# PSeitz/lz4_flex

Measured on AMD Instinct MI355X. Metric: MiB/s compress+decompress round trip, 1 GiB of 64 KiB JSON blocks per GPU (LZ4 block format), higher is better.
Workload: dtype u8

## Files before the change

lz4_flex_amd/csrc/lz4_compress_wave.hip:

```cpp
#include <hip/hip_runtime.h>
#include <stdint.h>

#include "lz4_device.h"

namespace lz4flex_dev {
namespace wave {

typedef __attribute__((address_space(3))) uint8_t lds_u8;
typedef __attribute__((address_space(3))) uint16_t lds_u16;
typedef __attribute__((address_space(3))) uint32_t lds_u32;
typedef uint32_t u32x4 __attribute__((ext_vector_type(4)));
typedef __attribute__((address_space(1))) uint8_t g_u8;
typedef __attribute__((address_space(1))) u32x4 g_u32x4;
typedef uint32_t u32x2 __attribute__((ext_vector_type(2)));
typedef __attribute__((address_space(1))) u32x2 g_u32x2;
typedef __attribute__((address_space(1))) uint32_t g_u32;
typedef __attribute__((address_space(1))) int32_t g_i32;

constexpr uint32_t WINDOW = 65536u;
#ifndef LZ4W_WORKERS
#define LZ4W_WORKERS 11
#endif
constexpr uint32_t WORKERS = LZ4W_WORKERS;
constexpr uint32_t GROUPS = WINDOW / 512u;
__host__ __device__ constexpr uint32_t seg_lo(uint32_t w) {
    if (WORKERS == 11u) {
        constexpr uint32_t lo[12] = {0u, 12u, 25u, 38u, 51u, 63u, 74u, 86u, 98u, 108u, 118u, 128u};
        return 512u * lo[w < 11u ? w : 11u];
    }
    if (WORKERS == 8u) {
        constexpr uint32_t lo[9] = {0u, 16u, 33u, 50u, 67u, 82u, 98u, 113u, 128u};
        return 512u * lo[w < 8u ? w : 8u];
    }
    return 512u * ((GROUPS * w) / WORKERS);
}
__host__ __device__ constexpr uint32_t seg_longest() {
    uint32_t m = 0u;
    for (uint32_t w = 0u; w < WORKERS; ++w) m = seg_lo(w + 1u) - seg_lo(w) > m ? seg_lo(w + 1u) - seg_lo(w) : m;
    return m;
}
constexpr uint32_t SEG = seg_longest();
constexpr uint32_t HIST = WINDOW / 2u;
__device__ __forceinline__ uint32_t seg_start(uint32_t j, uint32_t skip, uint32_t send) {
    if (send == 0u) return seg_lo(j) > skip ? seg_lo(j) : skip;
    if (j == 0u) return skip;
    if (j >= WORKERS) return send;
    const uint32_t span = send > skip ? send - skip : 0u;
    const uint32_t v = (skip + span * (seg_lo(j) / 512u) / 128u) & ~511u;
    return v > skip ? v : skip;
}

constexpr uint32_t CAP = 1024u;
constexpr uint32_t SKIPD = 64u;
constexpr uint32_t CARRY_SLOTS = 16u;
constexpr uint32_t CARRY_DWORDS = CARRY_SLOTS * 16u;
constexpr uint32_t CARRY_SPINS = 1u << 18;
constexpr uint32_t LONGK = 84u;
constexpr uint32_t NEARP = 20u;
constexpr uint32_t LONGN = 8u;
constexpr uint32_t HBITS = 12u;
constexpr uint32_t THREADS = 64u * (WORKERS + 1u);
#ifndef LZ4W_RING_SLOTS
#define LZ4W_RING_SLOTS 1
#endif
constexpr uint32_t RING_SLOTS = LZ4W_RING_SLOTS;
constexpr uint32_t TMP_OFF = 16u;
constexpr uint32_t CMP_OFF = TMP_OFF + 256u;
constexpr uint32_t WORKER_LDS = CMP_OFF + 256u;
constexpr uint32_t CHUNK = 1024u;
constexpr uint32_t CHUNK_SLOT = CHUNK + 16u;
constexpr uint32_t IDX_DEPTH = 4u;
constexpr uint32_t L_WIN = 0u;
constexpr uint32_t L_TAB = WINDOW + 64u;
constexpr uint32_t L_STG = L_TAB + (2u << HBITS);
constexpr uint32_t L_RING = L_STG + WORKERS * WORKER_LDS;
constexpr uint32_t L_META = L_RING + RING_SLOTS * CHUNK_SLOT;
constexpr uint32_t META_WORDS = 5u * WORKERS + 4u + 4u + 3u + 2u;
constexpr uint32_t LDS_BYTES = L_META + ((META_WORDS * 4u + 63u) & ~63u);
static_assert(LDS_BYTES <= 81920u, "two workgroups per CU");
static_assert(WORKERS >= 1u && WORKERS <= 15u && seg_lo(WORKERS) == WINDOW, "segments tile the window");
constexpr uint32_t SLOT_BYTES = 2u * WINDOW;
constexpr uint32_t BODY_STRIDE = (SEG + SEG / 128u + 255u) / 256u * 256u + 256u;
constexpr uint32_t WS_BYTES = 2u * SLOT_BYTES + WORKERS * BODY_STRIDE;
static_assert(WS_BYTES % 256u == 0u, "workspace slots stay 256 B aligned");
constexpr uint32_t STAGE_BYTES = WINDOW + 256u;
constexpr uint32_t STAGE_READ = WINDOW + 64u;

struct SegMeta {
    uint32_t has;
    uint32_t first_lit;
    uint32_t first_ml;
    uint32_t trail;
    uint32_t body_len;
};
struct BlkCarry { uint32_t out_pos, pend; };

__device__ __forceinline__ uint32_t dpp_wave_shr1(uint32_t v, uint32_t lane0) {
    return (uint32_t)__builtin_amdgcn_update_dpp((int)lane0, (int)v, 0x138, 0xf, 0xf, false);
}
__device__ __forceinline__ uint32_t dpp_wave_shl1(uint32_t v, uint32_t lane63) {
    return (uint32_t)__builtin_amdgcn_update_dpp((int)lane63, (int)v, 0x130, 0xf, 0xf, false);
}
#define LZ4W_DPP(v, ctrl, rmask) ((uint32_t)__builtin_amdgcn_update_dpp(0, (int)(v), (ctrl), (rmask), 0xf, false))
__device__ __forceinline__ uint32_t wave_incl_max(uint32_t v) {
    uint32_t t;
    t = LZ4W_DPP(v, 0x111, 0xf); v = v > t ? v : t;
    t = LZ4W_DPP(v, 0x112, 0xf); v = v > t ? v : t;
    t = LZ4W_DPP(v, 0x114, 0xf); v = v > t ? v : t;
    t = LZ4W_DPP(v, 0x118, 0xf); v = v > t ? v : t;
    t = LZ4W_DPP(v, 0x142, 0xa); v = v > t ? v : t;
    t = LZ4W_DPP(v, 0x143, 0xc); v = v > t ? v : t;
    return v;
}
__device__ __forceinline__ uint32_t wave_incl_add(uint32_t v) {
    v += LZ4W_DPP(v, 0x111, 0xf);
    v += LZ4W_DPP(v, 0x112, 0xf);
    v += LZ4W_DPP(v, 0x114, 0xf);
    v += LZ4W_DPP(v, 0x118, 0xf);
    v += LZ4W_DPP(v, 0x142, 0xa);
    v += LZ4W_DPP(v, 0x143, 0xc);
    return v;
}
__device__ __forceinline__ uint32_t rdlane(uint32_t v, uint32_t l) { return (uint32_t)__builtin_amdgcn_readlane((int)v, (int)l); }
__device__ __forceinline__ uint32_t uni(uint32_t v) { return (uint32_t)__builtin_amdgcn_readfirstlane((int)v); }
__device__ __forceinline__ uint64_t ld64l(const lds_u8* p) { uint64_t v; __builtin_memcpy(&v, (const void*)p, 8); return v; }
__device__ __forceinline__ uint32_t umin3(uint32_t a, uint32_t b, uint32_t c) { const uint32_t t = a < b ? a : b; return t < c ? t : c; }
__device__ __forceinline__ uint32_t ctz64(uint64_t x) { return (uint32_t)__builtin_ctzll(x); }
__device__ __forceinline__ uint32_t len_ext_bytes(uint32_t v) { return v >= 15u ? (v - 15u) / 255u + 1u : 0u; }

#ifndef LZ4W_NO_HWFFBL
__device__ __forceinline__ uint32_t ffbl(uint32_t x) { uint32_t r; asm("v_ffbl_b32 %0, %1" : "=v"(r) : "v"(x)); return r; }
#else
__device__ __forceinline__ uint32_t ffbl(uint32_t x) { return (uint32_t)(__ffs((int)x) - 1); }
#endif
template <typename G, typename T>
__device__ __forceinline__ G* uni_gptr(T* p) {
    const uint64_t v = (uint64_t)p;
    return (G*)(((uint64_t)uni((uint32_t)(v >> 32)) << 32) | uni((uint32_t)v));
}

struct ChunkRegs { u32x4 main; uint32_t extra; };

__device__ __forceinline__ void chunk_issue(ChunkRegs& r, const g_u8* __restrict__ gwin, uint32_t c, uint32_t lane) {
    const g_u8* pm = gwin + c * CHUNK + 16u * lane;
    const g_u8* pe = gwin + c * CHUNK + CHUNK;
#ifdef LZ4W_PLAIN_LOADS
    r.main = *reinterpret_cast<const g_u32x4*>(pm);
    r.extra = *reinterpret_cast<const g_u32*>(pe);
#else
    asm volatile("global_load_dwordx4 %0, %1, off ; lz4w-load" : "=v"(r.main) : "v"(pm) : "memory");
    asm volatile("global_load_dword %0, %1, off ; lz4w-load" : "=v"(r.extra) : "v"(pe) : "memory");
#endif
}
template <int N>
__device__ __forceinline__ void chunk_wait(ChunkRegs& r) {
#ifndef LZ4W_PLAIN_LOADS
    asm volatile("s_waitcnt vmcnt(%2) ; lz4w-wait %0 %1" : "+v"(r.main), "+v"(r.extra) : "n"(N) : "memory");
#endif
}
template <bool FULL>
__device__ __forceinline__ void index_chunk(const lds_u8* lp, lds_u16* tab, g_u8* __restrict__ cand_lane, uint32_t c, uint32_t act_n,
                                            uint32_t lane) {
#pragma unroll
    for (uint32_t g8 = 0; g8 < 2u; ++g8) {
        uint32_t h[8], e[8];
        uint64_t xr[8];
// ... 737 lines not shown
    u32x2 dn = *reinterpret_cast<const g_u32x2*>(cand_t + ((s0 >> 8) * 512u + lane * 8u));
#ifndef LZ4W_NO_PRIO
    const uint32_t prio_q = (s1 - s0 + 3u) / 4u;
    uint32_t prio_drop = s0 + prio_q, prio_lv = 3u;
    __builtin_amdgcn_s_setprio(3);
#endif
    for (uint32_t B0 = s0 & ~255u; B0 < s1; B0 += 256u) {
        const uint32_t dq0 = dn.x & 0xFFFFu, dq1 = dn.x >> 16, dq2 = dn.y & 0xFFFFu, dq3 = dn.y >> 16;
        dn = *reinterpret_cast<const g_u32x2*>(cand_t + (((B0 >> 8) + 1u) * 512u + lane * 8u));
#ifndef LZ4W_NO_PRIO
        if (B0 >= prio_drop) {
            prio_drop += prio_q;
            prio_lv = prio_lv != 0u ? prio_lv - 1u : 0u;
            if (prio_lv == 2u) __builtin_amdgcn_s_setprio(2);
            else if (prio_lv == 1u) __builtin_amdgcn_s_setprio(1);
            else __builtin_amdgcn_s_setprio(0);
        }
#endif
        if (superstep(UConst<4u>{}, B0, dq0, dq1, dq2, dq3)) continue;
#pragma unroll 1
        for (uint32_t hf = 0u; hf < 2u; ++hf) {
            const uint32_t bh = B0 + 128u * hf;
            if (bh >= s1) break;
            const uint32_t ta = hf ? dq2 : dq0, tb = hf ? dq3 : dq1;
            superstep(UConst<2u>{}, bh, ta, tb, 0u, 0u);
        }
    }
    st = encode_seqs(psq, psp, npend, body_, lane, st);
#ifndef LZ4W_NO_PRIO
    __builtin_amdgcn_s_setprio(3);
#endif
#ifdef LZ4W_PROF_STEPS
    if (prof_ && lane == 0u) {
        for (int i = 0; i < 5; ++i) atomicAdd(prof_ + 8 + i, (unsigned long long)pt[i]);
        atomicAdd(prof_ + 13, (unsigned long long)pn);
        atomicAdd(prof_ + 14, (unsigned long long)pt[5]);
        atomicAdd(prof_ + 15, (unsigned long long)pt[6]);
    }
#endif
    if (lane == 0u) {
        lds_u32* mp = (lds_u32*)(lds + L_META) + 5u * w;
        mp[0] = st.has; mp[1] = st.first_lit; mp[2] = st.first_ml; mp[3] = s1 - st.last_end; mp[4] = st.body_len;
    }
}

template <typename F>
__device__ __forceinline__ void put_bytes(g_u8* dst, uint32_t n, uint32_t lane, F f) {
    for (uint32_t i = lane; i < n; i += 64u) dst[i] = (uint8_t)f(i);
}
__device__ __forceinline__ void copy_bytes(g_u8* dst, const g_u8* src, uint32_t n, uint32_t lane) {
    uint32_t i = 0u;
    for (; i + 4096u <= n; i += 4096u) {
        u32x4 v[4];
#pragma unroll
        for (uint32_t j = 0; j < 4u; ++j) __builtin_memcpy(&v[j], (const void*)(src + i + 1024u * j + 16u * lane), 16);
#pragma unroll
        for (uint32_t j = 0; j < 4u; ++j) __builtin_memcpy((void*)(dst + i + 1024u * j + 16u * lane), &v[j], 16);
    }
    {
        u32x4 v[4];
#pragma unroll
        for (uint32_t j = 0; j < 4u; ++j) {
            const uint32_t o = i + 1024u * j + 16u * lane;
            v[j] = u32x4{0u, 0u, 0u, 0u};
            if (o + 16u <= n) __builtin_memcpy(&v[j], (const void*)(src + o), 16);
        }
#pragma unroll
        for (uint32_t j = 0; j < 4u; ++j) {
            const uint32_t o = i + 1024u * j + 16u * lane;
            if (o + 16u <= n) __builtin_memcpy((void*)(dst + o), &v[j], 16);
        }
    }
    const uint32_t done = i + ((n - i) & ~15u);
    if (done + lane < n) dst[done + lane] = src[done + lane];
}
__device__ __forceinline__ void put_len_header(g_u8* dst, uint32_t lit, uint32_t ml_nibble, uint32_t lane) {
    const uint32_t ne = len_ext_bytes(lit);
    put_bytes(dst, 1u + ne, lane, [&](uint32_t j) -> uint32_t {
        if (j == 0u) return ((lit < 15u ? lit : 15u) << 4) | ml_nibble;
        return (j < ne) ? 255u : (lit - 15u) % 255u;
    });
}

__device__ __attribute__((noinline)) void place_segment(lds_u8* lds, const uint8_t* __restrict__ gin_, uint32_t blk_len_, uint32_t win_idx_, bool last_win_,
                              uint32_t wl_, uint32_t wbase_, uint32_t wskip_, uint32_t send_, const uint8_t* body_, uint8_t* gout_, uint32_t carry_slot_, uint32_t w_, uint32_t lane,
                              uint32_t* out_len_, int32_t* status_, uint32_t* gcarry_, uint32_t iter_, uint32_t spins_max_, uint32_t runwin_) {
    const g_u8* __restrict__ gin = uni_gptr<const g_u8>(gin_);
    const uint32_t runwin = uni(runwin_);
    const g_u8* body = uni_gptr<const g_u8>(body_);
    g_u8* gout = uni_gptr<g_u8>(gout_);
    g_u32* out_len = uni_gptr<g_u32>(out_len_);
    g_i32* status = uni_gptr<g_i32>(status_);
    const uint32_t blk_len = uni(blk_len_), win_idx = uni(win_idx_), wl = uni(wl_), carry_slot = uni(carry_slot_), w = uni(w_);
    const uint32_t wbase = uni(wbase_), wskip = uni(wskip_);
    const uint32_t spins_max = uni(spins_max_);
    const bool last_win = uni((uint32_t)last_win_) != 0u;
    const uint32_t send = uni(send_);
    const lds_u32* mp = (const lds_u32*)(lds + L_META);
    lds_u32* cp = (lds_u32*)(lds + L_META) + 5u * WORKERS;
    g_u32* gcarry = uni_gptr<g_u32>(gcarry_);
    uint32_t out_pos = 0u, pend = 0u, poisoned = 0u;
    if (win_idx != 0u) {
        if (gcarry != nullptr) {
            const uint32_t iter = uni(iter_);
            typedef volatile __attribute__((address_space(3))) uint32_t lds_vu32;
            lds_vu32* box = (lds_vu32*)(lds + L_META) + 5u * WORKERS + 8u;
#ifndef LZ4W_NO_PRIO
            __builtin_amdgcn_s_setprio(0);
#endif
            if (w == WORKERS - 1u) {
                g_u32* sl = gcarry + 16u * (win_idx & (CARRY_SLOTS - 1u));
                uint32_t spins = 0u;
                while (__hip_atomic_load(sl + 2, __ATOMIC_ACQUIRE, __HIP_MEMORY_SCOPE_AGENT) != win_idx && ++spins < spins_max) __builtin_amdgcn_s_sleep(16);
                out_pos = __hip_atomic_load(sl, __ATOMIC_RELAXED, __HIP_MEMORY_SCOPE_AGENT);
                pend = __hip_atomic_load(sl + 1, __ATOMIC_RELAXED, __HIP_MEMORY_SCOPE_AGENT);
                if (spins >= spins_max) pend = 0x80000000u;
                if (lane == 0u) { box[0] = out_pos; box[1] = pend; }
                __builtin_amdgcn_fence(__ATOMIC_RELEASE, "workgroup");
                if (lane == 0u) box[2] = iter;
            } else {
                uint32_t spins = 0u;
                while (box[2] != iter && ++spins < (CARRY_SPINS << 4)) __builtin_amdgcn_s_sleep(2);
                __builtin_amdgcn_fence(__ATOMIC_ACQUIRE, "workgroup");
                out_pos = box[0];
                pend = spins >= (CARRY_SPINS << 4) ? 0x80000000u : box[1];
            }
#ifndef LZ4W_NO_PRIO
            __builtin_amdgcn_s_setprio(3);
#endif
            poisoned = pend >> 31;
            pend &= 0x7FFFFFFFu;
            if (poisoned) { out_pos = 0u; pend = 0u; }
            out_pos = uni(out_pos); pend = uni(pend); poisoned = uni(poisoned);
        } else {
            out_pos = cp[2u * (carry_slot ^ 1u)]; pend = cp[2u * (carry_slot ^ 1u) + 1u];
        }
    }
    auto seg_at = [&](uint32_t j) -> uint32_t {
        const uint32_t v = runwin ? (j == 0u ? wskip : wl) : seg_start(j, wskip, send);
        return v < wl ? v : wl;
    };
    auto seg_len = [&](uint32_t j) -> uint32_t { return seg_at(j + 1u) - seg_at(j); };
    for (uint32_t j = 0; j < w; ++j) {
        const uint32_t sl = seg_len(j);
        if (mp[5u * j] != 0u) {
            const uint32_t L = pend + mp[5u * j + 1u];
            out_pos += 1u + len_ext_bytes(L) + L + mp[5u * j + 4u];
            pend = mp[5u * j + 3u];
        } else {
            pend += sl;
        }
    }
    const uint32_t sl = seg_len(w);
    const uint32_t abs0 = wbase + seg_at(w);
    if (gcarry != nullptr && w == WORKERS - 1u && !last_win && lane == 0u) {
        uint32_t eo = out_pos, ep = pend;
        if (mp[5u * w] != 0u) {
            const uint32_t L = pend + mp[5u * w + 1u];
            eo += 1u + len_ext_bytes(L) + L + mp[5u * w + 4u];
            ep = mp[5u * w + 3u];
        } else {
            ep += sl;
        }
        g_u32* so = gcarry + 16u * ((win_idx + 1u) & (CARRY_SLOTS - 1u));
        __hip_atomic_store(so, eo, __ATOMIC_RELAXED, __HIP_MEMORY_SCOPE_AGENT);
        __hip_atomic_store(so + 1, ep | (poisoned << 31), __ATOMIC_RELAXED, __HIP_MEMORY_SCOPE_AGENT);
        __hip_atomic_store(so + 2, win_idx + 1u, __ATOMIC_RELEASE, __HIP_MEMORY_SCOPE_AGENT);
    }
    if (mp[5u * w] != 0u) {
        const uint32_t fl = mp[5u * w + 1u], L = pend + fl, ml = mp[5u * w + 2u] - 4u, bl = mp[5u * w + 4u];
        put_len_header(gout + out_pos, L, ml < 15u ? ml : 15u, lane);
        out_pos += 1u + len_ext_bytes(L);
        copy_bytes(gout + out_pos, gin + (abs0 + fl - L), L, lane);
        out_pos += L;
        copy_bytes(gout + out_pos, body, bl, lane);
        out_pos += bl;
        pend = mp[5u * w + 3u];
    } else {
        pend += sl;
    }
    if (w == WORKERS - 1u) {
        if (last_win) {
            put_len_header(gout + out_pos, pend, 0u, lane);
            out_pos += 1u + len_ext_bytes(pend);
            copy_bytes(gout + out_pos, gin + (blk_len - pend), pend, lane);
            out_pos += pend;
            if (lane == 0u) { *out_len = poisoned ? 0u : out_pos; *status = poisoned ? 66  : 0; }
        } else if (lane == 0u) {
            cp[2u * carry_slot] = out_pos;
            cp[2u * carry_slot + 1u] = pend;
        }
    }
}

__device__ __attribute__((noinline)) void load_window(const uint8_t* __restrict__ g_, uint32_t wl_, uint32_t rd_n_, lds_u8* lds, uint32_t tid) {
    constexpr uint32_t NT = 64u * WORKERS;
    const g_u8* __restrict__ g = uni_gptr<const g_u8>(g_);
    const uint32_t wl = uni(wl_), rd_n = uni(rd_n_);
    const uint32_t mis = (uint32_t)((16u - ((uintptr_t)g & 15u)) & 15u);
    const uint32_t head = mis < wl ? mis : wl;
    if (tid < head) lds[L_WIN + tid] = g[tid];
    const uint32_t nvec = (wl - head) / 16u;
    const g_u8* gp = g + head + 16u * tid;
    lds_u8* lp = lds + L_WIN + head + 16u * tid;
#pragma unroll 1
    for (uint32_t i0 = 0; i0 < nvec; i0 += 4u * NT) {
        u32x4 v[4];
#pragma unroll
        for (uint32_t j = 0; j < 4u; ++j) {
            v[j] = u32x4{0u, 0u, 0u, 0u};
            if (i0 + tid + NT * j < nvec) v[j] = *reinterpret_cast<const g_u32x4*>(gp + 16u * NT * j);
        }
#pragma unroll
        for (uint32_t j = 0; j < 4u; ++j)
            if (i0 + tid + NT * j < nvec) __builtin_memcpy((void*)(lp + 16u * NT * j), &v[j], 16);
        gp += 64u * NT;
        lp += 64u * NT;
    }
    const uint32_t done = head + 16u * nvec;
    if (tid < wl - done) lds[L_WIN + done + tid] = g[done + tid];
    if (tid < 64u) lds[L_WIN + wl + tid] = wl + tid < rd_n ? g[wl + tid] : (uint8_t)0;
}

struct WaveArgs : CompressArgs {
    const uint8_t* shared_dict;
    uint32_t shared_len;
    uint32_t shared_hs;
    uint32_t shared_keep;
    uint8_t* digest;
};
template <class A> constexpr bool IS_SHARED = __is_same(A, WaveArgs);
struct SetArgs : CompressArgs {
    DictSetArgs set;
};
template <class A> constexpr bool IS_SET = __is_same(A, SetArgs);
template <class A> constexpr bool HAS_DIGEST = IS_SHARED<A> || IS_SET<A>;
struct Item {
    uint32_t blk, win, nwin, len, skip, hist, slide;
    uint32_t sub;
    uint32_t dct;
    uint32_t did;
    uint64_t in_off;
};
__device__ __forceinline__ uint32_t win_stride(const Item& t) { return t.slide != 0u ? t.slide : WINDOW; }
__device__ __forceinline__ uint32_t win_base(const Item& t) {
    if (t.sub != 0u) return 0u;
    return (t.win + 1u == t.nwin && t.len > WINDOW) ? t.len - WINDOW : t.win * win_stride(t);
}
__device__ __forceinline__ uint32_t win_from(const Item& t) {
    if (t.sub != 0u) return t.win * t.sub;
    return t.win == 0u ? t.hist : (t.win - 1u) * win_stride(t) + WINDOW;
}
__device__ __forceinline__ uint32_t win_skip(const Item& t) { return win_from(t) - win_base(t); }
__device__ __forceinline__ uint32_t win_len(const Item& t) {
    if (t.sub != 0u) return t.win + 1u == t.nwin ? t.len : (t.win + 1u) * t.sub;
    const uint32_t base = win_base(t);
    return t.len > base ? (t.len - base < WINDOW ? t.len - base : WINDOW) : 0u;
}
__device__ __forceinline__ uint32_t win_send(const Item& t) { return t.sub != 0u ? win_len(t) : (t.slide != 0u ? WINDOW : 0u); }
template <class A>
__device__ __forceinline__ void item_load(const A& a, Item& it) {
    it.win = 0u; it.nwin = 0u; it.len = 0u; it.skip = 0u; it.hist = 0u; it.slide = 0u; it.sub = 0u; it.dct = 0u; it.did = 0u; it.in_off = 0ull;
    if (it.blk >= a.n) return;
    const uint32_t len = a.in_len[it.blk];
    const uint32_t cap = a.out_cap[it.blk];
    uint32_t h = (a.flags != nullptr && (a.flags[it.blk] >> 8) >= HIST && len != 0u && len <= 0xFFFFFFFFu - HIST) ? HIST : 0u;
    uint32_t dl = a.dict_len != nullptr ? a.dict_len[it.blk] : 0u;
    if constexpr (IS_SHARED<A>) dl = a.shared_len;
    if constexpr (IS_SET<A>) {
        const uint32_t id = a.set.dict_id[it.blk];
        if (id != DICT_ID_NONE) {
            if (id >= a.set.k) { it.skip = 2u; it.nwin = 1u; return; }
            dl = a.set.table[id].len;
            it.did = id;
// ... 2 lines not shown
    if (dl != 0u) {
        h = dl < HIST ? dl : HIST;
        if ((a.flags != nullptr && a.flags[it.blk] != 0u) || len > 0xFFFFFFFFu - h) { it.skip = 2u; it.nwin = 1u; return; }
        it.dct = 1u;
    }
    it.hist = h;
    it.len = len + h;
    it.in_off = a.in_off[it.blk] - h;
    it.slide = h != 0u ? HIST : ((a.slide != 0u && len > WINDOW) ? a.slide : 0u);
    it.nwin = it.slide != 0u ? (it.len <= WINDOW ? 1u : 1u + (it.len - WINDOW + it.slide - 1u) / it.slide)
                      : (len == 0u ? 1u : (uint32_t)(((uint64_t)len + WINDOW - 1u) / WINDOW));
    if (a.sub >= 2u && a.sub <= 4u && h == 0u && len <= WINDOW) {
        const uint32_t q = ((WINDOW + a.sub - 1u) / a.sub + 511u) & ~511u;
        if (len > q) { it.sub = q; it.nwin = (len + q - 1u) / q; }
    }
    const uint64_t need = 20ull + (uint64_t)len * 110ull / 100ull;
    if ((uint64_t)cap < need) { it.skip = 1u; it.nwin = 1u; }
}
template <class A>
__device__ __forceinline__ const uint8_t* win_src(const A& a, const Item& t, const uint8_t* stg) {
    return t.dct ? stg : a.in_base + t.in_off + (size_t)win_base(t);
}
__device__ __forceinline__ uint32_t win_rd(const Item& t) {
    const uint32_t r = t.len - win_base(t);
    return t.dct && r > STAGE_READ ? STAGE_READ : r;
}
template <class A>
__device__ __forceinline__ void item_seek(const A& a, Item& it, int32_t redo) {
    if (redo != 0)
        while (it.blk < a.n && a.status[it.blk] != redo) it.blk += gridDim.x;
    item_load(a, it);
}
template <class A>
__device__ __forceinline__ void item_next_block(const A& a, Item& it, int32_t redo) {
    if (it.win + 1u < it.nwin) { it.win += 1u; return; }
    it.blk += gridDim.x;
    item_seek(a, it, redo);
}
template <class A>
__device__ __forceinline__ void item_draw(const A& a, uint32_t* wctr, uint32_t b0, uint32_t& ob, uint32_t& ow) {
    const uint32_t n = a.n;
    uint32_t b = b0;
    const uint32_t tries = n < 8u ? n : 8u;
    for (uint32_t t = 0; t < tries; ++t) {
        Item q;
        q.blk = b;
        item_load(a, q);
        const uint32_t w = atomicAdd(wctr + b, 1u);
        if (w < q.nwin) { ob = b; ow = w; return; }
        b = b + 1u == n ? 0u : b + 1u;
    }
    ob = n; ow = 0u;
}

struct RunGeom { uint32_t ok, ms, me; };
__device__ __forceinline__ RunGeom run_geom(const Item& t) {
    RunGeom g;
    const uint32_t base = win_base(t), wl = win_len(t), skip = win_skip(t);
    g.ms = skip > 1u ? skip : 1u;
    uint32_t me = t.len >= 5u + base ? t.len - 5u - base : 0u;
    me = me < wl ? me : wl;
    g.me = me < 65535u ? me : 65535u;
    const uint32_t act_abs = t.len >= 12u ? t.len - 11u : 0u;
#ifdef LZ4W_NO_RUN_WINDOWS
    g.ok = 0u;
#else
    g.ok = (wl >= RUN_MIN && !t.skip && base + g.ms < act_abs && g.me >= g.ms + 4u) ? 1u : 0u;
#endif
    return g;
}

__device__ __forceinline__ const uint8_t* item_digest(const WaveArgs& a, const Item&) { return a.digest; }
__device__ __forceinline__ uint32_t item_hs(const WaveArgs& a, const Item&) { return a.shared_hs; }
__device__ __forceinline__ uint32_t* item_counter(const WaveArgs& a) { return (uint32_t*)(a.digest + DG_HDR) + 2; }
__device__ __forceinline__ const DictSetRec* set_rec(const SetArgs& a, const Item& t) { return uni_gptr<const DictSetRec>(a.set.table) + uni(t.did); }
__device__ __forceinline__ const uint8_t* item_digest(const SetArgs& a, const Item& t) { return uni_gptr<const uint8_t>(set_rec(a, t)->digest); }
__device__ __forceinline__ uint32_t item_hs(const SetArgs& a, const Item& t) { return a.set.use != 0u ? uni(set_rec(a, t)->hs) : 0u; }
__device__ __forceinline__ uint32_t* item_counter(const SetArgs& a) { return a.set.counter; }
__device__ __forceinline__ uint32_t keep_tag(const WaveArgs& a, const Item&) { return a.shared_keep != 0u ? 1u : 0u; }
__device__ __forceinline__ bool keep_hit(const WaveArgs&, const Item&, uint32_t kept) { return kept != 0u; }
__device__ __forceinline__ uint32_t keep_tag(const SetArgs& a, const Item& t) { return a.set.use != 0u ? t.did + 1u : 0u; }
__device__ __forceinline__ bool keep_hit(const SetArgs&, const Item& t, uint32_t kept) { return kept == t.did + 1u; }

template <class A>
__device__ __forceinline__ void wave_body(const A& a, uint8_t* __restrict__ ws, uint32_t* __restrict__ carry,
                                          unsigned long long* __restrict__ prof, const int32_t redo, const uint32_t carry_spins) {
    extern __shared__ __attribute__((aligned(16))) uint8_t dyn_lds[];
    lds_u8* lds = (lds_u8*)dyn_lds;
    if ((uint32_t)(uintptr_t)lds != 0u) {
        for (uint32_t b = blockIdx.x * THREADS + threadIdx.x; b < a.n; b += gridDim.x * THREADS) { a.out_len[b] = 0u; a.status[b] = 66; }
        return;
    }
    const uint32_t lane = threadIdx.x & 63u;
    const uint32_t w = uni(threadIdx.x >> 6);
#ifdef LZ4W_EXP_IDX_PRIO
    if (w == WORKERS) __builtin_amdgcn_s_setprio(LZ4W_EXP_IDX_PRIO);
#endif
    uint8_t* my_ws = ws + (size_t)blockIdx.x * WS_BYTES;
    uint8_t* slots = my_ws;
    uint8_t* bodies = my_ws + 2u * SLOT_BYTES;
    uint8_t* stg = a.stage + (size_t)blockIdx.x * STAGE_BYTES;

    const bool wmode = carry != nullptr;
    lds_u32* giq = (lds_u32*)(lds + L_META) + 5u * WORKERS + 4u;
    uint32_t* wctr = wmode ? carry + CARRY_DWORDS * (size_t)a.n : nullptr;
    Item it, ix;
    if (threadIdx.x == 0u) giq[6] = 0u;
    if (wmode) {
        if (threadIdx.x == 0u) {
            uint32_t b = a.n, wn = 0u;
            item_draw(a, wctr, blockIdx.x % a.n, b, wn);
            giq[0] = b; giq[1] = wn;
        }
        __syncthreads();
        it.blk = giq[0];
        item_load(a, it);
        it.win = giq[1];
        ix.blk = a.n;
        item_load(a, ix);
    } else {
        it.blk = blockIdx.x;
        item_seek(a, it, redo);
        ix = it;
        item_next_block(a, ix, redo);
    }
    if (it.blk >= a.n) return;
    uint32_t k = 0u;

    lds_u32* run_flag = (lds_u32*)(lds + L_META) + 5u * WORKERS + 11u;
    [[maybe_unused]] uint32_t tail_kept = 0u;
    auto do_stage = [&](const Item& t) {
        const uint32_t base = win_base(t);
        const uint32_t nrd = win_rd(t);
        if constexpr (HAS_DIGEST<A>) {
            const uint32_t from = (t.win == 0u && keep_hit(a, t, tail_kept)) ? (t.hist & ~15u) : 0u;
            stage_window(item_digest(a, t) + DG_TAIL, a.in_base + t.in_off, base + from, nrd - from, t.hist, stg + from, lane);
            tail_kept = t.win == 0u ? keep_tag(a, t) : 0u;
            return;
        } else {
        const uint8_t* tail = a.dict_base + a.dict_off[t.blk] + (a.dict_len[t.blk] - t.hist);
        stage_window(tail, a.in_base + t.in_off, base, nrd, t.hist, stg, lane);
        }
    };
    auto do_index = [&](const Item& t, uint32_t slot, bool stage) {
        if (t.skip) { if (lane == 0u) run_flag[slot] = 0u; return; }
        if (t.dct && stage) do_stage(t);
        const uint32_t base = win_base(t), wl = win_len(t);
        const uint32_t act_abs = t.len >= 12u ? t.len - 11u : 0u;
        const uint32_t act_n = act_abs > base ? (act_abs - base < wl ? act_abs - base : wl) : 0u;
        const RunGeom rg = run_geom(t);
        if constexpr (HAS_DIGEST<A>) {
            const uint32_t hs = (IS_SHARED<A> || t.dct != 0u) ? item_hs(a, t) : 0u;
            if (t.win == 0u && hs != 0u && act_n >= hs) {
                const uint32_t run = index_window<true>(win_src(a, t, stg), wl, act_n, win_rd(t), slots + (size_t)slot * SLOT_BYTES, lds, lane, rg.ok,
                                                        DigestRef<true>{item_digest(a, t), hs});
                if (redo == 0 && lane == 0u)
                    __hip_atomic_fetch_add(item_counter(a), 1u, __ATOMIC_RELAXED, __HIP_MEMORY_SCOPE_AGENT);
                if (lane == 0u) run_flag[slot] = run;
                return;
            }
        }
        const uint32_t run = index_window<false>(win_src(a, t, stg), wl, act_n, win_rd(t), slots + (size_t)slot * SLOT_BYTES, lds, lane, rg.ok, DigestRef<false>{});
        if (lane == 0u) run_flag[slot] = run;
    };
    auto do_load = [&](const Item& t) {
        if (t.skip) return;
        load_window(win_src(a, t, stg), win_len(t), win_rd(t), lds, threadIdx.x);
    };

    uint64_t t_prev = prof ? __builtin_readcyclecounter() : 0ull;
    uint64_t t_acc[7] = {0ull, 0ull, 0ull, 0ull, 0ull, 0ull, 0ull};
    auto tick = [&](uint32_t slot) {
        if (prof) {
            const uint64_t t = __builtin_readcyclecounter();
#pragma unroll
            for (uint32_t i = 0; i < 7u; ++i) t_acc[i] += i == slot ? t - t_prev : 0ull;
            t_prev = t;
        }
    };
    if (it.dct && !it.skip) {
        if (w == WORKERS) do_stage(it);
        __syncthreads();
    }
    if (w == WORKERS) { do_index(it, 0u, false); tick(0u); }
    else { do_load(it); tick(5u); }
    __syncthreads();
    tick(w == WORKERS ? 1u : 6u);
    if (wmode) {
        if (threadIdx.x == 0u) {
            uint32_t b2 = a.n, w2 = 0u;
            item_draw(a, wctr, it.blk, b2, w2);
            giq[2] = b2; giq[3] = w2;
        }
        __syncthreads();
        ix.blk = giq[2];
        item_load(a, ix);
        ix.win = giq[3];
        __syncthreads();
    }
    for (;;) {
        const uint32_t wl = win_len(it);
        const bool last_win = it.win + 1u == it.nwin;
        if (w == WORKERS) {
            if (ix.blk < a.n) do_index(ix, (k + 1u) & 1u, true);
        } else if (!it.skip) {
            const uint32_t base = win_base(it), skip = win_skip(it);
            uint32_t s0 = seg_start(w, skip, win_send(it));
            uint32_t s1 = seg_start(w + 1u, skip, win_send(it));
            s0 = s0 < wl ? s0 : wl;
            s1 = s1 < wl ? s1 : wl;
            const uint32_t act_abs = it.len >= 12u ? it.len - 11u : 0u;
            const uint32_t mfl_end = act_abs > base ? act_abs - base : 0u;
            uint32_t mend = it.len >= 5u ? it.len - 5u : 0u;
            mend = mend > base ? mend - base : 0u;
            mend = mend < s1 ? mend : s1;
            mend = mend < 65535u ? mend : 65535u;
            if (run_flag[k & 1u] != 0u) {
                const RunGeom rg = run_geom(it);
                lds_u32* mp = (lds_u32*)(lds + L_META) + 5u * w;
                if (w == 0u) {
                    emit_generic(bodies, 0u, 0u, 0u, 1u, rg.me - rg.ms, 1u, lane);
                    if (lane == 0u) { mp[0] = 1u; mp[1] = rg.ms - skip; mp[2] = rg.me - rg.ms; mp[3] = wl - rg.me; mp[4] = 2u + len_ext_bytes(rg.me - rg.ms - 4u); }
                } else if (lane == 0u) {
                    mp[0] = 0u; mp[1] = 0u; mp[2] = 0u; mp[3] = 0u; mp[4] = 0u;
                }
            } else if (s0 < s1) {
                match_segment(slots + (size_t)(k & 1u) * SLOT_BYTES, bodies + (size_t)w * BODY_STRIDE, w, lane, s0, s1, mfl_end, mend, prof);
            } else if (lane == 0u) {
                lds_u32* mp = (lds_u32*)(lds + L_META) + 5u * w;
                mp[0] = 0u; mp[1] = 0u; mp[2] = 0u; mp[3] = 0u; mp[4] = 0u;
            }
        }
        tick(w == WORKERS ? 0u : 2u);
        __syncthreads();
        tick(w == WORKERS ? 1u : 3u);
        if (wmode && threadIdx.x == 0u) {
            uint32_t b2 = a.n, w2 = 0u;
            if (ix.blk < a.n) item_draw(a, wctr, ix.blk, b2, w2);
            giq[2] = b2; giq[3] = w2;
        }
        if (w != WORKERS) {
            if (it.skip) {
                if (threadIdx.x == 0u) { a.out_len[it.blk] = 0u; a.status[it.blk] = ((HAS_DIGEST<A> || a.dict_len != nullptr) && it.skip == 2u) ? LZ4FLEX_DEV_E_INVALID_ARG : LZ4FLEX_DEV_E_OUTPUT_TOO_SMALL; }
            } else {
                place_segment(lds, a.in_base + it.in_off, it.len, it.win, last_win, wl, win_base(it), win_skip(it), win_send(it), bodies + (size_t)w * BODY_STRIDE,
                              a.out_base + a.out_off[it.blk], k & 1u, w, lane, a.out_len + it.blk, a.status + it.blk,
                              wmode ? carry + CARRY_DWORDS * (size_t)it.blk : nullptr, k + 1u, carry_spins, run_flag[k & 1u]);
            }
        }
        tick(w == WORKERS ? 1u : 4u);
        if (prof && threadIdx.x == 0u) atomicAdd(prof + 7, 1ull);
        it = ix;
        k += 1u;
        if (it.blk >= a.n) {
            if (prof && lane == 0u)
                for (uint32_t i = 0; i < 7u; ++i)
                    if (t_acc[i] != 0ull) atomicAdd(prof + i, (unsigned long long)t_acc[i]);
#ifdef LZ4W_PROF_WORKERS
            if (prof && lane == 0u && w < WORKERS) atomicAdd(prof + 16u + w, (unsigned long long)t_acc[2]);
#endif
            break;
        }
        if (w != WORKERS) do_load(it);
        tick(w == WORKERS ? 1u : 5u);
        __syncthreads();
        tick(w == WORKERS ? 1u : 6u);
        if (wmode) { ix.blk = giq[2]; item_load(a, ix); ix.win = giq[3]; }
        else item_next_block(a, ix, redo);
    }
}

__device__ __forceinline__ CompressArgs no_dicts(CompressArgs a) {
    a.dict_base = nullptr; a.dict_off = nullptr; a.dict_len = nullptr;
    return a;
}
__device__ __forceinline__ WaveArgs only_shared(const CompressArgs& a, const SharedDictArgs& sh) {
    WaveArgs r;
    static_cast<CompressArgs&>(r) = no_dicts(a);
    r.flags = nullptr;
    r.shared_dict = sh.dict; r.shared_len = sh.len; r.shared_hs = sh.hs; r.shared_keep = sh.keep; r.digest = sh.digest;
    return r;
}
__device__ __forceinline__ SetArgs only_set(const CompressArgs& a, const DictSetArgs& st) {
    SetArgs r;
    static_cast<CompressArgs&>(r) = no_dicts(a);
    r.flags = nullptr;
    r.set = st;
    return r;
}
__global__ void __launch_bounds__(THREADS) __attribute__((amdgpu_waves_per_eu(6, 6))) lz4_compress_wave_kernel(const CompressArgs a, uint8_t* __restrict__ ws,
                                                                    uint32_t* __restrict__ carry, unsigned long long* __restrict__ prof, uint32_t carry_spins) {
    wave_body(no_dicts(a), ws, carry, prof, 0, carry_spins);
}
__global__ void __launch_bounds__(THREADS) __attribute__((amdgpu_waves_per_eu(6, 6))) lz4_compress_wave_redo_kernel(const CompressArgs a, uint8_t* __restrict__ ws,
                                                                                                                     int32_t redo) {
    wave_body(no_dicts(a), ws, nullptr, nullptr, redo, CARRY_SPINS);
}
__global__ void __launch_bounds__(THREADS) __attribute__((amdgpu_waves_per_eu(6, 6))) lz4_compress_wave_dict_kernel(const CompressArgs a, uint8_t* __restrict__ ws,
                                                                    uint32_t* __restrict__ carry, unsigned long long* __restrict__ prof, uint32_t carry_spins) {
    wave_body(a, ws, carry, prof, 0, carry_spins);
}
__global__ void __launch_bounds__(THREADS) __attribute__((amdgpu_waves_per_eu(6, 6))) lz4_compress_wave_dict_redo_kernel(const CompressArgs a, uint8_t* __restrict__ ws,
                                                                                                                          int32_t redo) {
    wave_body(a, ws, nullptr, nullptr, redo, CARRY_SPINS);
}
__global__ void __launch_bounds__(THREADS) __attribute__((amdgpu_waves_per_eu(6, 6))) lz4_compress_wave_shared_kernel(const CompressArgs a, const SharedDictArgs sh,
                                                                    uint8_t* __restrict__ ws, uint32_t* __restrict__ carry, unsigned long long* __restrict__ prof, uint32_t carry_spins) {
    wave_body(only_shared(a, sh), ws, carry, prof, 0, carry_spins);
}
__global__ void __launch_bounds__(THREADS) __attribute__((amdgpu_waves_per_eu(6, 6))) lz4_compress_wave_shared_redo_kernel(const CompressArgs a, const SharedDictArgs sh,
                                                                                                                            uint8_t* __restrict__ ws, int32_t redo) {
    wave_body(only_shared(a, sh), ws, nullptr, nullptr, redo, CARRY_SPINS);
}
__global__ void __launch_bounds__(THREADS) __attribute__((amdgpu_waves_per_eu(6, 6))) lz4_wave_set_kernel(const CompressArgs a, const DictSetArgs st,
                                                                    uint8_t* __restrict__ ws, uint32_t* __restrict__ carry, unsigned long long* __restrict__ prof, uint32_t carry_spins) {
    wave_body(only_set(a, st), ws, carry, prof, 0, carry_spins);
}
__global__ void __launch_bounds__(THREADS) __attribute__((amdgpu_waves_per_eu(6, 6))) lz4_wave_set_redo_kernel(const CompressArgs a, const DictSetArgs st,
                                                                                                                         uint8_t* __restrict__ ws, int32_t redo) {
    wave_body(only_set(a, st), ws, nullptr, nullptr, redo, CARRY_SPINS);
}

}

static size_t wave_stage_at(int n_workgroups) { return ((size_t)n_workgroups * (wave::WS_BYTES + wave::CARRY_DWORDS * 4u + 4u) + 255u) & ~(size_t)255u; }
static size_t wave_digest_at(int n_workgroups) { return wave_stage_at(n_workgroups) + (size_t)n_workgroups * wave::STAGE_BYTES; }
size_t compress_wave_workspace_bytes(int n_workgroups) { return wave_digest_at(n_workgroups) + wave::DIGEST_BYTES; }
const uint32_t* compress_wave_shared_counter(const void* workspace, int n_workgroups) {
    return (const uint32_t*)((const uint8_t*)workspace + wave_digest_at(n_workgroups) + wave::DG_HDR) + 2;
}

size_t compress_wave_digest_bytes() { return wave::DIGEST_BYTES; }
uint32_t compress_wave_digest_hs(uint32_t h) { return wave::digest_hs(h); }
size_t compress_wave_digest_scratch_bytes() { return wave::DIGEST_SCRATCH; }
hipError_t launch_dict_set_digests(const DictSetRec* table, uint32_t k, uint8_t* cand_scratch, hipStream_t s) {
    if (k == 0u) return hipSuccess;
    hipLaunchKernelGGL(wave::lz4_set_digest_kernel, dim3(k), dim3(64), (2u << wave::HBITS) + wave::CHUNK_SLOT, s, table, cand_scratch);
    return hipGetLastError();
}

// ... 78 lines not shown
```

Measured before the change: 217,900.

## Defer segment output copies to next iteration with ticket-based work stealing

Splits place_segment into resolve_window, which computes each segment's output offsets and records them in a double-buffered LDS record, and copy_segment, which writes the literals and match bodies. The copies for window k now run during iteration k+1 after matching, handed out to worker waves through an LDS atomic ticket. Waves that finish matching early pick up the copy work, so the serial placement phase between barriers is meant to shrink and the load across waves to even out. Small copies are batched into register-held pieces so loads are issued before stores. In exchange, the body workspace is doubled to hold two sets, LDS metadata grows, and a final drain step is added after the loop, with extra synchronisation complexity.

```diff
diff --git a/lz4_flex_amd/csrc/lz4_compress_wave.hip b/lz4_flex_amd/csrc/lz4_compress_wave.hip
--- a/lz4_flex_amd/csrc/lz4_compress_wave.hip
+++ b/lz4_flex_amd/csrc/lz4_compress_wave.hip
@@ -75,13 +75,19 @@
 constexpr uint32_t L_STG = L_TAB + (2u << HBITS);
 constexpr uint32_t L_RING = L_STG + WORKERS * WORKER_LDS;
 constexpr uint32_t L_META = L_RING + RING_SLOTS * CHUNK_SLOT;
-constexpr uint32_t META_WORDS = 5u * WORKERS + 4u + 4u + 3u + 2u;
+constexpr uint32_t M_TICKET = 5u * WORKERS + 13u;
+constexpr uint32_t M_REC = M_TICKET + 1u;
+constexpr uint32_t REC_SEG = 7u;
+constexpr uint32_t REC_UNI = REC_SEG * WORKERS;
+constexpr uint32_t REC_WORDS = REC_UNI + 18u;
+constexpr uint32_t META_WORDS = M_REC + 2u * REC_WORDS;
 constexpr uint32_t LDS_BYTES = L_META + ((META_WORDS * 4u + 63u) & ~63u);
 static_assert(LDS_BYTES <= 81920u, "two workgroups per CU");
 static_assert(WORKERS >= 1u && WORKERS <= 15u && seg_lo(WORKERS) == WINDOW, "segments tile the window");
 constexpr uint32_t SLOT_BYTES = 2u * WINDOW;
 constexpr uint32_t BODY_STRIDE = (SEG + SEG / 128u + 255u) / 256u * 256u + 256u;
-constexpr uint32_t WS_BYTES = 2u * SLOT_BYTES + WORKERS * BODY_STRIDE;
+constexpr uint32_t BODY_SET = WORKERS * BODY_STRIDE;
+constexpr uint32_t WS_BYTES = 2u * SLOT_BYTES + 2u * BODY_SET;
 static_assert(WS_BYTES % 256u == 0u, "workspace slots stay 256 B aligned");
 constexpr uint32_t STAGE_BYTES = WINDOW + 256u;
 constexpr uint32_t STAGE_READ = WINDOW + 64u;
@@ -985,15 +991,30 @@
     });
 }
 
-__device__ __attribute__((noinline)) void place_segment(lds_u8* lds, const uint8_t* __restrict__ gin_, uint32_t blk_len_, uint32_t win_idx_, bool last_win_,
-                              uint32_t wl_, uint32_t wbase_, uint32_t wskip_, uint32_t send_, const uint8_t* body_, uint8_t* gout_, uint32_t carry_slot_, uint32_t w_, uint32_t lane,
+constexpr uint32_t RU_COUNT = 0u;
+constexpr uint32_t RU_GIN = 1u;
+constexpr uint32_t RU_BLK_LEN = 3u;
+constexpr uint32_t RU_WIN_IDX = 4u;
+constexpr uint32_t RU_LAST_WIN = 5u;
+constexpr uint32_t RU_WL = 6u;
+constexpr uint32_t RU_WBASE = 7u;
+constexpr uint32_t RU_WSKIP = 8u;
+constexpr uint32_t RU_SEND = 9u;
+constexpr uint32_t RU_GOUT = 10u;
+constexpr uint32_t RU_RUNWIN = 12u;
+constexpr uint32_t RU_POISONED = 13u;
+constexpr uint32_t RU_OUT_LEN = 14u;
+constexpr uint32_t RU_STATUS = 16u;
+static_assert(RU_STATUS + 2u == REC_WORDS - REC_UNI, "the record holds the uniform values");
+__device__ __forceinline__ uint32_t seg_at(uint32_t j, uint32_t runwin, uint32_t wl, uint32_t wskip, uint32_t send) {
+    const uint32_t v = runwin ? (j == 0u ? wskip : wl) : seg_start(j, wskip, send);
+    return v < wl ? v : wl;
+}
+
+__device__ __attribute__((noinline)) void resolve_window(lds_u8* lds, uint32_t rec_, const uint8_t* __restrict__ gin_, uint32_t blk_len_, uint32_t win_idx_, bool last_win_,
+                              uint32_t wl_, uint32_t wbase_, uint32_t wskip_, uint32_t send_, uint8_t* gout_, uint32_t carry_slot_, uint32_t w_, uint32_t lane,
                               uint32_t* out_len_, int32_t* status_, uint32_t* gcarry_, uint32_t iter_, uint32_t spins_max_, uint32_t runwin_) {
-    const g_u8* __restrict__ gin = uni_gptr<const g_u8>(gin_);
     const uint32_t runwin = uni(runwin_);
-    const g_u8* body = uni_gptr<const g_u8>(body_);
-    g_u8* gout = uni_gptr<g_u8>(gout_);
-    g_u32* out_len = uni_gptr<g_u32>(out_len_);
-    g_i32* status = uni_gptr<g_i32>(status_);
     const uint32_t blk_len = uni(blk_len_), win_idx = uni(win_idx_), wl = uni(wl_), carry_slot = uni(carry_slot_), w = uni(w_);
     const uint32_t wbase = uni(wbase_), wskip = uni(wskip_);
     const uint32_t spins_max = uni(spins_max_);
@@ -1001,6 +1022,7 @@
     const uint32_t send = uni(send_);
     const lds_u32* mp = (const lds_u32*)(lds + L_META);
     lds_u32* cp = (lds_u32*)(lds + L_META) + 5u * WORKERS;
+    lds_u32* rec = (lds_u32*)(lds + L_META) + uni(rec_);
     g_u32* gcarry = uni_gptr<g_u32>(gcarry_);
     uint32_t out_pos = 0u, pend = 0u, poisoned = 0u;
     if (win_idx != 0u) {
@@ -1039,60 +1061,123 @@
             out_pos = cp[2u * (carry_slot ^ 1u)]; pend = cp[2u * (carry_slot ^ 1u) + 1u];
         }
     }
-    auto seg_at = [&](uint32_t j) -> uint32_t {
-        const uint32_t v = runwin ? (j == 0u ? wskip : wl) : seg_start(j, wskip, send);
-        return v < wl ? v : wl;
+    uint32_t m_has = 0u, m_fl = 0u, m_ml = 0u, m_tr = 0u, m_bl = 0u;
+    if (lane < WORKERS) { m_has = mp[5u * lane]; m_fl = mp[5u * lane + 1u]; m_ml = mp[5u * lane + 2u]; m_tr = mp[5u * lane + 3u]; m_bl = mp[5u * lane + 4u]; }
+    auto behind = [&](uint32_t j, uint32_t& op, uint32_t& pd) {
+        if (rdlane(m_has, j) != 0u) {
+            const uint32_t L = pd + rdlane(m_fl, j);
+            op += 1u + len_ext_bytes(L) + L + rdlane(m_bl, j);
+            pd = rdlane(m_tr, j);
+        } else {
+            pd += seg_at(j + 1u, runwin, wl, wskip, send) - seg_at(j, runwin, wl, wskip, send);
+        }
     };
-    auto seg_len = [&](uint32_t j) -> uint32_t { return seg_at(j + 1u) - seg_at(j); };
-    for (uint32_t j = 0; j < w; ++j) {
-        const uint32_t sl = seg_len(j);
-        if (mp[5u * j] != 0u) {
-            const uint32_t L = pend + mp[5u * j + 1u];
-            out_pos += 1u + len_ext_bytes(L) + L + mp[5u * j + 4u];
-            pend = mp[5u * j + 3u];
+    for (uint32_t j = 0; j < w; ++j) behind(j, out_pos, pend);
+    if (lane == w) {
+        lds_u32* sg = rec + REC_SEG * w;
+        sg[0] = out_pos; sg[1] = pend; sg[2] = m_has; sg[3] = m_fl; sg[4] = m_ml; sg[5] = m_tr; sg[6] = m_bl;
+    }
+    if (w == 0u && lane == 0u) {
+        lds_u32* ru = rec + REC_UNI;
+        const uint64_t pin = (uint64_t)gin_, pout = (uint64_t)gout_, plen = (uint64_t)out_len_, pst = (uint64_t)status_;
+        ru[RU_COUNT] = WORKERS;
+        ru[RU_GIN] = (uint32_t)pin; ru[RU_GIN + 1u] = (uint32_t)(pin >> 32);
+        ru[RU_BLK_LEN] = blk_len; ru[RU_WIN_IDX] = win_idx; ru[RU_LAST_WIN] = last_win ? 1u : 0u;
+        ru[RU_WL] = wl; ru[RU_WBASE] = wbase; ru[RU_WSKIP] = wskip; ru[RU_SEND] = send;
+        ru[RU_GOUT] = (uint32_t)pout; ru[RU_GOUT + 1u] = (uint32_t)(pout >> 32);
+        ru[RU_RUNWIN] = runwin; ru[RU_POISONED] = poisoned;
+        ru[RU_OUT_LEN] = (uint32_t)plen; ru[RU_OUT_LEN + 1u] = (uint32_t)(plen >> 32);
+        ru[RU_STATUS] = (uint32_t)pst; ru[RU_STATUS + 1u] = (uint32_t)(pst >> 32);
+    }
+    uint32_t eo = out_pos, ep = pend;
+    if (w == WORKERS - 1u && !last_win) behind(w, eo, ep);
+    if (w == WORKERS - 1u && !last_win && lane == 0u) {
+        if (gcarry != nullptr) {
+            g_u32* so = gcarry + 16u * ((win_idx + 1u) & (CARRY_SLOTS - 1u));
+            __hip_atomic_store(so, eo, __ATOMIC_RELAXED, __HIP_MEMORY_SCOPE_AGENT);
+            __hip_atomic_store(so + 1, ep | (poisoned << 31), __ATOMIC_RELAXED, __HIP_MEMORY_SCOPE_AGENT);
+            __hip_atomic_store(so + 2, win_idx + 1u, __ATOMIC_RELEASE, __HIP_MEMORY_SCOPE_AGENT);
         } else {
-            pend += sl;
-        }
-    }
-    const uint32_t sl = seg_len(w);
-    const uint32_t abs0 = wbase + seg_at(w);
-    if (gcarry != nullptr && w == WORKERS - 1u && !last_win && lane == 0u) {
-        uint32_t eo = out_pos, ep = pend;
-        if (mp[5u * w] != 0u) {
-            const uint32_t L = pend + mp[5u * w + 1u];
-            eo += 1u + len_ext_bytes(L) + L + mp[5u * w + 4u];
-            ep = mp[5u * w + 3u];
-        } else {
-            ep += sl;
-        }
-        g_u32* so = gcarry + 16u * ((win_idx + 1u) & (CARRY_SLOTS - 1u));
-        __hip_atomic_store(so, eo, __ATOMIC_RELAXED, __HIP_MEMORY_SCOPE_AGENT);
-        __hip_atomic_store(so + 1, ep | (poisoned << 31), __ATOMIC_RELAXED, __HIP_MEMORY_SCOPE_AGENT);
-        __hip_atomic_store(so + 2, win_idx + 1u, __ATOMIC_RELEASE, __HIP_MEMORY_SCOPE_AGENT);
-    }
-    if (mp[5u * w] != 0u) {
-        const uint32_t fl = mp[5u * w + 1u], L = pend + fl, ml = mp[5u * w + 2u] - 4u, bl = mp[5u * w + 4u];
+            cp[2u * carry_slot] = eo;
+            cp[2u * carry_slot + 1u] = ep;
+        }
+    }
+}
+
+constexpr uint32_t PIECE = 1024u;
+struct Piece { u32x4 v; uint32_t t; };
+__device__ __forceinline__ Piece piece_load(const g_u8* src, uint32_t n, uint32_t lane) {
+    Piece p;
+    p.v = u32x4{0u, 0u, 0u, 0u};
+    p.t = 0u;
+    if (16u * lane + 16u <= n) __builtin_memcpy(&p.v, (const void*)(src + 16u * lane), 16);
+    if ((n & ~15u) + lane < n) p.t = src[(n & ~15u) + lane];
+    return p;
+}
+__device__ __forceinline__ void piece_store(g_u8* dst, uint32_t n, uint32_t lane, const Piece& p) {
+    if (16u * lane + 16u <= n) __builtin_memcpy((void*)(dst + 16u * lane), &p.v, 16);
+    if ((n & ~15u) + lane < n) dst[(n & ~15u) + lane] = (uint8_t)p.t;
+}
+
+__device__ __attribute__((noinline)) void copy_segment(lds_u8* lds, uint32_t rec_, uint32_t t_, const uint8_t* bodies_, uint32_t lane) {
+    const lds_u32* rec = (const lds_u32*)(lds + L_META) + uni(rec_);
+    const uint32_t t = uni(t_);
+    const lds_u32* sg = rec + REC_SEG * t;
+    const lds_u32* ru = rec + REC_UNI;
+    auto rd = [&](const lds_u32* p) -> uint32_t { return uni(*p); };
+    auto rd_ptr = [&](const lds_u32* p) -> uint64_t { return ((uint64_t)rd(p + 1) << 32) | rd(p); };
+    const g_u8* __restrict__ gin = (const g_u8*)rd_ptr(ru + RU_GIN);
+    g_u8* gout = (g_u8*)rd_ptr(ru + RU_GOUT);
+    const g_u8* body = uni_gptr<const g_u8>(bodies_) + (size_t)t * BODY_STRIDE;
+    const uint32_t wl = rd(ru + RU_WL), wbase = rd(ru + RU_WBASE), wskip = rd(ru + RU_WSKIP), send = rd(ru + RU_SEND), runwin = rd(ru + RU_RUNWIN);
+    uint32_t out_pos = rd(sg), pend = rd(sg + 1);
+    const uint32_t abs0 = wbase + seg_at(t, runwin, wl, wskip, send);
+    const bool has = rd(sg + 2) != 0u;
+    const uint32_t fl = rd(sg + 3), L = pend + fl, ml = rd(sg + 4) - 4u, bl = has ? rd(sg + 6) : 0u;
+    const uint32_t lit_at = out_pos + 1u + len_ext_bytes(L), body_at = lit_at + L;
+    if (has) {
         put_len_header(gout + out_pos, L, ml < 15u ? ml : 15u, lane);
-        out_pos += 1u + len_ext_bytes(L);
-        copy_bytes(gout + out_pos, gin + (abs0 + fl - L), L, lane);
-        out_pos += L;
-        copy_bytes(gout + out_pos, body, bl, lane);
-        out_pos += bl;
-        pend = mp[5u * w + 3u];
+        out_pos = body_at + bl;
+        pend = rd(sg + 5);
     } else {
-        pend += sl;
-    }
-    if (w == WORKERS - 1u) {
-        if (last_win) {
-            put_len_header(gout + out_pos, pend, 0u, lane);
-            out_pos += 1u + len_ext_bytes(pend);
-            copy_bytes(gout + out_pos, gin + (blk_len - pend), pend, lane);
-            out_pos += pend;
-            if (lane == 0u) { *out_len = poisoned ? 0u : out_pos; *status = poisoned ? 66  : 0; }
-        } else if (lane == 0u) {
-            cp[2u * carry_slot] = out_pos;
-            cp[2u * carry_slot + 1u] = pend;
-        }
+        pend += seg_at(t + 1u, runwin, wl, wskip, send) - seg_at(t, runwin, wl, wskip, send);
+    }
+    const bool fin = t == WORKERS - 1u && rd(ru + RU_LAST_WIN) != 0u;
+    const uint32_t blk_len = rd(ru + RU_BLK_LEN);
+    const uint32_t fin_at = out_pos + 1u + len_ext_bytes(pend);
+    if (fin) {
+        put_len_header(gout + out_pos, pend, 0u, lane);
+        out_pos = fin_at + pend;
+    }
+    const bool lit_small = has && L <= PIECE, fin_small = fin && pend <= PIECE;
+    if (has && !lit_small) copy_bytes(gout + lit_at, gin + (abs0 + fl - L), L, lane);
+    if (fin && !fin_small) copy_bytes(gout + fin_at, gin + (blk_len - pend), pend, lane);
+    Piece pl = piece_load(gin + (abs0 + fl - L), lit_small ? L : 0u, lane);
+    Piece pf = piece_load(gin + (blk_len - pend), fin_small ? pend : 0u, lane);
+    const uint32_t bh = bl < 4096u ? bl : 4096u, be = bh & ~15u;
+    u32x4 bv[4];
+#pragma unroll
+    for (uint32_t j = 0; j < 4u; ++j) {
+        const uint32_t o = 1024u * j + 16u * lane;
+        bv[j] = u32x4{0u, 0u, 0u, 0u};
+        if (o + 16u <= bh) __builtin_memcpy(&bv[j], (const void*)(body + o), 16);
+    }
+    uint32_t bt = 0u;
+    if (be + lane < bh) bt = body[be + lane];
+    piece_store(gout + lit_at, lit_small ? L : 0u, lane, pl);
+#pragma unroll
+    for (uint32_t j = 0; j < 4u; ++j) {
+        const uint32_t o = 1024u * j + 16u * lane;
+        if (o + 16u <= bh) __builtin_memcpy((void*)(gout + body_at + o), &bv[j], 16);
+    }
+    if (be + lane < bh) gout[body_at + be + lane] = (uint8_t)bt;
+    piece_store(gout + fin_at, fin_small ? pend : 0u, lane, pf);
+    if (bl > 4096u) copy_bytes(gout + body_at + 4096u, body + 4096u, bl - 4096u, lane);
+    if (fin) {
+        const uint32_t poisoned = rd(ru + RU_POISONED);
+        g_u32* out_len = (g_u32*)rd_ptr(ru + RU_OUT_LEN);
+        g_i32* status = (g_i32*)rd_ptr(ru + RU_STATUS);
+        if (lane == 0u) { *out_len = poisoned ? 0u : out_pos; *status = poisoned ? 66  : 0; }
     }
 }
 
@@ -1261,6 +1346,7 @@
 __device__ __forceinline__ uint32_t keep_tag(const SetArgs& a, const Item& t) { return a.set.use != 0u ? t.did + 1u : 0u; }
 __device__ __forceinline__ bool keep_hit(const SetArgs&, const Item& t, uint32_t kept) { return kept == t.did + 1u; }
 
+constexpr uint32_t PROF_RESOLVE = 27u;
 template <class A>
 __device__ __forceinline__ void wave_body(const A& a, uint8_t* __restrict__ ws, uint32_t* __restrict__ carry,
                                           unsigned long long* __restrict__ prof, const int32_t redo, const uint32_t carry_spins) {
@@ -1284,7 +1370,13 @@
     lds_u32* giq = (lds_u32*)(lds + L_META) + 5u * WORKERS + 4u;
     uint32_t* wctr = wmode ? carry + CARRY_DWORDS * (size_t)a.n : nullptr;
     Item it, ix;
-    if (threadIdx.x == 0u) giq[6] = 0u;
+    lds_u32* meta = (lds_u32*)(lds + L_META);
+    if (threadIdx.x == 0u) {
+        giq[6] = 0u;
+        meta[M_TICKET] = 0u;
+        meta[M_REC + REC_UNI + RU_COUNT] = 0u;
+        meta[M_REC + REC_WORDS + REC_UNI + RU_COUNT] = 0u;
+    }
     if (wmode) {
         if (threadIdx.x == 0u) {
             uint32_t b = a.n, wn = 0u;
@@ -1348,12 +1440,12 @@
     };
 
     uint64_t t_prev = prof ? __builtin_readcyclecounter() : 0ull;
-    uint64_t t_acc[7] = {0ull, 0ull, 0ull, 0ull, 0ull, 0ull, 0ull};
+    uint64_t t_acc[8] = {0ull, 0ull, 0ull, 0ull, 0ull, 0ull, 0ull, 0ull};
     auto tick = [&](uint32_t slot) {
         if (prof) {
             const uint64_t t = __builtin_readcyclecounter();
 #pragma unroll
-            for (uint32_t i = 0; i < 7u; ++i) t_acc[i] += i == slot ? t - t_prev : 0ull;
+            for (uint32_t i = 0; i < 8u; ++i) t_acc[i] += i == slot ? t - t_prev : 0ull;
             t_prev = t;
         }
     };
@@ -1398,19 +1490,44 @@
                 const RunGeom rg = run_geom(it);
                 lds_u32* mp = (lds_u32*)(lds + L_META) + 5u * w;
                 if (w == 0u) {
-                    emit_generic(bodies, 0u, 0u, 0u, 1u, rg.me - rg.ms, 1u, lane);
+                    emit_generic(bodies + (size_t)(k & 1u) * BODY_SET, 0u, 0u, 0u, 1u, rg.me - rg.ms, 1u, lane);
                     if (lane == 0u) { mp[0] = 1u; mp[1] = rg.ms - skip; mp[2] = rg.me - rg.ms; mp[3] = wl - rg.me; mp[4] = 2u + len_ext_bytes(rg.me - rg.ms - 4u); }
                 } else if (lane == 0u) {
                     mp[0] = 0u; mp[1] = 0u; mp[2] = 0u; mp[3] = 0u; mp[4] = 0u;
                 }
             } else if (s0 < s1) {
-                match_segment(slots + (size_t)(k & 1u) * SLOT_BYTES, bodies + (size_t)w * BODY_STRIDE, w, lane, s0, s1, mfl_end, mend, prof);
+                match_segment(slots + (size_t)(k & 1u) * SLOT_BYTES, bodies + (size_t)(k & 1u) * BODY_SET + (size_t)w * BODY_STRIDE, w, lane, s0, s1, mfl_end, mend, prof);
             } else if (lane == 0u) {
                 lds_u32* mp = (lds_u32*)(lds + L_META) + 5u * w;
                 mp[0] = 0u; mp[1] = 0u; mp[2] = 0u; mp[3] = 0u; mp[4] = 0u;
             }
         }
         tick(w == WORKERS ? 0u : 2u);
+        if (w != WORKERS) {
+            const uint32_t rec = M_REC + ((k + 1u) & 1u) * REC_WORDS;
+            const uint32_t cnt = uni(meta[rec + REC_UNI + RU_COUNT]);
+            auto draw = [&]() -> uint32_t {
+                uint32_t t = 0u;
+                if (lane == 0u) t = __hip_atomic_fetch_add(meta + M_TICKET, 1u, __ATOMIC_RELAXED, __HIP_MEMORY_SCOPE_WORKGROUP);
+                return uni(t);
+            };
+            uint32_t t = cnt != 0u ? draw() : cnt;
+            if (t < cnt) {
+#ifndef LZ4W_NO_PRIO
+                __builtin_amdgcn_s_setprio(0);
+#endif
+                __builtin_amdgcn_fence(__ATOMIC_ACQUIRE, "workgroup");
+                do {
+                    copy_segment(lds, rec, cnt - 1u - t, bodies + (size_t)((k + 1u) & 1u) * BODY_SET, lane);
+                    t = draw();
+                } while (t < cnt);
+#ifndef LZ4W_NO_PRIO
+                __builtin_amdgcn_s_setprio(3);
+#endif
+            }
+            __builtin_amdgcn_fence(__ATOMIC_RELEASE, "workgroup");
+            tick(4u);
+        }
         __syncthreads();
         tick(w == WORKERS ? 1u : 3u);
         if (wmode && threadIdx.x == 0u) {
@@ -1419,22 +1536,34 @@
             giq[2] = b2; giq[3] = w2;
         }
         if (w != WORKERS) {
+            const uint32_t rec = M_REC + (k & 1u) * REC_WORDS;
+            if (threadIdx.x == 0u) meta[M_TICKET] = 0u;
             if (it.skip) {
-                if (threadIdx.x == 0u) { a.out_len[it.blk] = 0u; a.status[it.blk] = ((HAS_DIGEST<A> || a.dict_len != nullptr) && it.skip == 2u) ? LZ4FLEX_DEV_E_INVALID_ARG : LZ4FLEX_DEV_E_OUTPUT_TOO_SMALL; }
+                if (threadIdx.x == 0u) {
+                    a.out_len[it.blk] = 0u; a.status[it.blk] = ((HAS_DIGEST<A> || a.dict_len != nullptr) && it.skip == 2u) ? LZ4FLEX_DEV_E_INVALID_ARG : LZ4FLEX_DEV_E_OUTPUT_TOO_SMALL;
+                    meta[rec + REC_UNI + RU_COUNT] = 0u;
+                }
             } else {
-                place_segment(lds, a.in_base + it.in_off, it.len, it.win, last_win, wl, win_base(it), win_skip(it), win_send(it), bodies + (size_t)w * BODY_STRIDE,
-                              a.out_base + a.out_off[it.blk], k & 1u, w, lane, a.out_len + it.blk, a.status + it.blk,
-                              wmode ? carry + CARRY_DWORDS * (size_t)it.blk : nullptr, k + 1u, carry_spins, run_flag[k & 1u]);
+                resolve_window(lds, rec, a.in_base + it.in_off, it.len, it.win, last_win, wl, win_base(it), win_skip(it), win_send(it),
+                               a.out_base + a.out_off[it.blk], k & 1u, w, lane, a.out_len + it.blk, a.status + it.blk,
+                               wmode ? carry + CARRY_DWORDS * (size_t)it.blk : nullptr, k + 1u, carry_spins, run_flag[k & 1u]);
             }
         }
-        tick(w == WORKERS ? 1u : 4u);
+        tick(w == WORKERS ? 1u : 7u);
         if (prof && threadIdx.x == 0u) atomicAdd(prof + 7, 1ull);
         it = ix;
         k += 1u;
         if (it.blk >= a.n) {
+            __syncthreads();
+            tick(w == WORKERS ? 1u : 6u);
+            const uint32_t lrec = M_REC + ((k + 1u) & 1u) * REC_WORDS;
+            if (w != WORKERS && meta[lrec + REC_UNI + RU_COUNT] != 0u) {
+                copy_segment(lds, lrec, w, bodies + (size_t)((k + 1u) & 1u) * BODY_SET, lane);
+                tick(4u);
+            }
             if (prof && lane == 0u)
-                for (uint32_t i = 0; i < 7u; ++i)
-                    if (t_acc[i] != 0ull) atomicAdd(prof + i, (unsigned long long)t_acc[i]);
+                for (uint32_t i = 0; i < 8u; ++i)
+                    if (t_acc[i] != 0ull) atomicAdd(prof + (i < 7u ? i : PROF_RESOLVE), (unsigned long long)t_acc[i]);
 #ifdef LZ4W_PROF_WORKERS
             if (prof && lane == 0u && w < WORKERS) atomicAdd(prof + 16u + w, (unsigned long long)t_acc[2]);
 #endif
```

New measurement: 221,200, median of 6. 1.02x the previous value.
